# songhayeong/aes-fhe

Measured on AMD Instinct MI355X. Metric: AES-128 blocks/sec (homomorphic full round) at N=2^16, L=30; 1/2/4/8 MI355X, higher is better.
Workload: dtype u64

## Files before the change

aes-fhe_amd/csrc/bconv_cols.h:

```cpp
#pragma once
#include "bconv_mfma.h"
#include "ntt256f.h"

namespace aesfhe {

__device__ __forceinline__ void cols256_stages_store(double (&x)[16], double q, double qi, bool big, const double* tg,
                                                     const double* tws, double* s, u64* out, int b, int cl, int c) {
#pragma unroll
    for (int st = 0; st < 4; st++) {
        const int m = 1 << st, hh = 8 >> st;
        if (big && st == 2) {
#pragma unroll
            for (int a = 0; a < 16; a++) x[a] = fred(x[a], q, qi);
        }
#pragma unroll
        for (int a = 0; a < 16; a++) {
            if (a & hh) continue;
            const int ti = m + (a >> (4 - st));
            ct_f(x[a], x[a + hh], tg[ti], q, qi);
        }
    }
#pragma unroll
    for (int a = 0; a < 16; a++) s[(a * 16 + b) * kPadF + cl] = x[a];
    __syncthreads();
    const int ap = b;
#pragma unroll
    for (int bb = 0; bb < 16; bb++) x[bb] = s[(ap * 16 + bb) * kPadF + cl];
#pragma unroll
    for (int st = 4; st < 8; st++) {
        const int m = 1 << st, hh = 128 >> st;
        if (big && (st & 1) == 0) {
#pragma unroll
            for (int bb = 0; bb < 16; bb++) x[bb] = fred(x[bb], q, qi);
        }
#pragma unroll
        for (int bb = 0; bb < 16; bb++) {
            if (bb & hh) continue;
            ct_f(x[bb], x[bb + hh], tws[m + ap * (m >> 4) + (bb >> (8 - st))], q, qi);
        }
    }
#pragma unroll
    for (int bb = 0; bb < 16; bb++) st_d(&out[(ap * 16 + bb) * 256 + c], x[bb]);
}

template <int NSTEP, bool YIN, bool VC = false, int PF = 1, int TT = 4, int LT = 2, int MODE = 0>
__global__ __launch_bounds__(256, TT == 4 ? 2 : 3) void k_bconv_cols(BconvArgs a, Tabs T, int ntile) {
    static_assert(TT == 4 || TT == 2, "4 or 2 targets per workgroup");
    static_assert(LT == 1 || LT == 2, "1 or 2 LDS tiles");
    __shared__ double s[LT][256 * kPadF];
    __shared__ double tws[TT][256];
    const int tid = threadIdx.x, lane = tid & 63, w = tid >> 6, c = lane & 31, h = lane >> 5;
    const int cl = tid & 15, b = tid >> 4;
    const int id = blockIdx.x, x8 = id & 7, j = id >> 3;
    const int tile = j % ntile, u = (j / ntile) * 8 + x8;
    const int bx = u & 15, z = u >> 4, zb = z / a.nc, zc = z - zb * a.nc;
    const int logN = T.logN;
    const u64* src = a.src + (long)zb * a.sbs + (long)zc * a.scs;
    u64* dst = a.dst + (long)zb * a.dbs + (long)zc * a.dcs;
    auto limb_of = [&](int tau) { return tau < a.skip0 ? tau : tau + a.skipn; };
    auto pid_of = [&](int tl) { return tl <= a.tl_l ? tl : a.Lp1 + tl - a.tl_l - 1; };
    const int tau0 = TT * tile;
    const int nlive = min(TT, a.nt - tau0);
#pragma unroll
    for (int m = 0; m < TT; m++)
        if (m < nlive) tws[m][tid] = T.psid[((long)pid_of(limb_of(tau0 + m)) << logN) + tid];
    bc_v4i af[NSTEP];
    {
        const int row = lane & 31, ta = row >> 3, pb = (row & 3) + 4 * ((row >> 2) & 1);
        const int tau = tau0 + ta;
        const bc_v4i* ap =
            (const bc_v4i*)(a.tab + ((long)(ta < TT && tau < a.nt ? pid_of(limb_of(tau)) : 0) * 8 + pb) * kBconvKT + 16 * h);
#pragma unroll
        for (int st = 0; st < NSTEP; st++) af[st] = ap[2 * st];
    }
    const u64* sp[NSTEP][2];
    double sq[NSTEP][2], sf[NSTEP][2];
#pragma unroll
    for (int st = 0; st < NSTEP; st++)
#pragma unroll
        for (int uu = 0; uu < 2; uu++) {
            const int sl = 4 * st + 2 * h + uu;
            const int i = sl < a.ns ? sl : 0;
            sp[st][uu] = src + ((long)i << logN) + bx * 16 + (c & 15);
            if (!YIN) {
                const int pid = i < a.s_nq ? a.s_q0 + i : a.s_p0 + i - a.s_nq;
                sq[st][uu] = (double)a.qall[pid];
                sf[st][uu] = a.sinvf[i];
            }
        }
    double xv[TT][16];
    double eq[TT], eqi[TT], ew32[TT], ef32[TT], ecr[TT];
#pragma unroll
    for (int m = 0; m < TT; m++) {
        const int pid = tau0 + m < a.nt ? pid_of(limb_of(tau0 + m)) : 0;
        const double* pc = a.pc + 4 * pid;
        eq[m] = pc[0], eqi[m] = pc[1], ew32[m] = pc[2], ef32[m] = pc[3], ecr[m] = a.corr[pid];
    }
    double ev[VC ? 4 * NSTEP : 1];
#pragma unroll
    for (int sl = 0; sl < (VC ? 4 * NSTEP : 0); sl++) ev[sl] = a.einv[sl];
    u64 raw[PF + 1][NSTEP][2][2];
    auto load = [&](u64 (&r)[NSTEP][2][2], int ar) {
#pragma unroll
        for (int st = 0; st < NSTEP; st++)
#pragma unroll
            for (int uu = 0; uu < 2; uu++)
#pragma unroll
                for (int g = 0; g < 2; g++) r[st][uu][g] = sp[st][uu][(16 * ar + 4 * w + 2 * g + (c >> 4)) * 256];
    };
#pragma unroll
    for (int p = 0; p < PF; p++) load(raw[p], p);
#pragma unroll
    for (int ar = 0; ar < 16; ar++) {
        if (ar + PF < 16) load(raw[(ar + PF) % (PF + 1)], ar + PF);
        bc_v4i bf[2][NSTEP];
        double ys[2][NSTEP][2];
#pragma unroll
        for (int st = 0; st < NSTEP; st++)
#pragma unroll
            for (int uu = 0; uu < 2; uu++)
#pragma unroll
                for (int g = 0; g < 2; g++) {
                    u64 yb = PF ? raw[ar % (PF + 1)][st][uu][g] : sp[st][uu][(16 * ar + 4 * w + 2 * g + (c >> 4)) * 256];
                    if (!YIN) {
                        const double q = sq[st][uu], f = sf[st][uu];
                        double y = fmul_rem(u2d(yb), tw_w(f, q), f, q);
                        y = y < 0.0 ? y + q : y;
                        yb = (u64)__double_as_longlong(y + 4503599627370496.0) & 0xFFFFFFFFFFFFFULL;
                    }
                    if (VC) ys[g][st][uu] = u2d(yb);
                    bf[g][st][2 * uu] = (int)(unsigned)yb ^ (int)0x80808080;
                    bf[g][st][2 * uu + 1] = (int)(unsigned)(yb >> 32) ^ (int)0x80808080;
                }
        if constexpr (VC) {
            double yl[NSTEP][2][2];
#pragma unroll
            for (int st = 0; st < NSTEP; st++)
#pragma unroll
                for (int uu = 0; uu < 2; uu++) swap_halves(ys[0][st][uu], ys[1][st][uu], yl[st][uu][0], yl[st][uu][1]);
            double sum = 0.0;
#pragma unroll
            for (int st = 0; st < NSTEP; st++)
#pragma unroll
                for (int hh = 0; hh < 2; hh++)
#pragma unroll
                    for (int uu = 0; uu < 2; uu++) {
                        const int sl = 4 * st + 2 * hh + uu;
                        sum = sum + yl[st][uu][hh] * ev[sl];
                    }
            const int vown = (int)__builtin_rint(sum);
            const auto pr = __builtin_amdgcn_permlane32_swap((unsigned)vown, (unsigned)vown, false, false);
            const int voth = (int)(h ? pr[0] : pr[1]);
#pragma unroll
            for (int st = 0; st < NSTEP; st++)
#pragma unroll
                for (int uu = 0; uu < 2; uu++)
                    if (4 * st + 2 * h + uu == a.ns) {
#pragma unroll
                        for (int g = 0; g < 2; g++) {
                            bf[g][st][2 * uu] = ((g == h ? vown : voth) & 0xff) ^ (int)0x80808080;
                            bf[g][st][2 * uu + 1] = (int)0x80808080;
                        }
                    }
        }
        if constexpr (MODE == 2) {
#pragma unroll
            for (int m = 0; m < TT; m++) xv[m][ar] = (double)(bf[0][0][0] & 0xffffff) + (double)(bf[1][NSTEP - 1][3] & 0xff);
            continue;
        }
        bc_v16i acc[2];
#pragma unroll
        for (int g = 0; g < 2; g++) {
            acc[g] = bc_v16i{};
#pragma unroll
            for (int st = 0; st < NSTEP; st++) acc[g] = __builtin_amdgcn_mfma_i32_32x32x32_i8(af[st], bf[g][st], acc[g], 0, 0, 0);
        }
#pragma unroll
        for (int m = 0; m < TT; m++) {
            if (m >= nlive) break;
            double part[2];
#pragma unroll
            for (int g = 0; g < 2; g++) {
                const int p01 = acc[g][4 * m] + acc[g][4 * m + 1] * 256, p23 = acc[g][4 * m + 2] + acc[g][4 * m + 3] * 256;
                part[g] = __builtin_fma((double)p23, 65536.0, (double)p01);
            }
            double lo, hi;
            swap_halves(part[0], part[1], lo, hi);
            xv[m][ar] = fred(lo + fmul_rem(hi, ew32[m], ef32[m], eq[m]) + ecr[m], eq[m], eqi[m]);
        }
    }
    __syncthreads();
    if constexpr (MODE == 1) {
#pragma unroll
        for (int m = 0; m < TT; m++) {
            if (m >= nlive) break;
            u64* o = dst + ((long)limb_of(tau0 + m) << logN);
#pragma unroll
            for (int ar = 0; ar < 16; ar++) st_d(&o[(ar * 16 + b) * 256 + bx * 16 + cl], xv[m][ar]);
        }
        return;
    }
#pragma unroll
    for (int m = 0; m < TT; m++) {
        if (m >= nlive) break;
        if (LT == 1 && m > 0) __syncthreads();
        const int tl = limb_of(tau0 + m), pid = pid_of(tl);
        const double q = (double)T.q[pid], qi = T.qinv[pid];
        cols256_stages_store(xv[m], q, qi, q >= kBigPrime, T.psid + ((long)pid << logN), tws[m], s[m % LT],
                             dst + ((long)tl << logN), b, cl, bx * 16 + cl);
    }
}

}
```

aes-fhe_amd/csrc/ks_fused.h:

```cpp
#pragma once
#include "kernels_ops.h"
#include "ntt256f.h"

namespace aesfhe {

__device__ __forceinline__ int r8p(int e) { return e + (e >> 3); }

__device__ __forceinline__ void wave_lds_sync() {
    __builtin_amdgcn_fence(__ATOMIC_RELEASE, "wavefront");
    __builtin_amdgcn_wave_barrier();
    __builtin_amdgcn_fence(__ATOMIC_ACQUIRE, "wavefront");
}

__device__ __forceinline__ void row_ntt8_stages(double (&x)[8], double* sr, int L, int rt, const double* W, double q,
                                                double qi, bool big);
__device__ __forceinline__ void row_ntt8_fwd(double (&x)[8], const u64* rp, double* sr, int L, int rt,
                                             const double* W, double q, double qi, bool big) {
#pragma unroll
    for (int r = 0; r < 8; r++) x[r] = ld_d(&rp[L + 32 * r]);
    row_ntt8_stages(x, sr, L, rt, W, q, qi, big);
}
__device__ __forceinline__ void row_ntt8_stages(double (&x)[8], double* sr, int L, int rt, const double* W, double q,
                                                double qi, bool big) {
#pragma unroll
    for (int st = 0; st < 3; st++) {
        const int ml = 1 << st, h = 4 >> st;
        if (big && (st & 1) == 0) {
#pragma unroll
            for (int r = 0; r < 8; r++) x[r] = fred(x[r], q, qi);
        }
        const int base = ml * rt;
#pragma unroll
        for (int j = 0; j < ml; j++) {
            const double w = W[base + j];
#pragma unroll
            for (int k = 0; k < h; k++) ct_f(x[j * 2 * h + k], x[j * 2 * h + k + h], w, q, qi);
        }
    }
#pragma unroll
    for (int r = 0; r < 8; r++) sr[r8p(L + 32 * r)] = x[r];
    wave_lds_sync();
    const int eb = 32 * (L >> 2) + (L & 3);
#pragma unroll
    for (int r = 0; r < 8; r++) x[r] = sr[r8p(eb + 4 * r)];
#pragma unroll
    for (int st = 3; st < 6; st++) {
        const int ml = 1 << st, h = 4 >> (st - 3), nj = ml >> 3;
        if (big && (st & 1) == 0) {
#pragma unroll
            for (int r = 0; r < 8; r++) x[r] = fred(x[r], q, qi);
        }
        const int base = ml * rt + (L >> 2) * nj;
#pragma unroll
        for (int j = 0; j < nj; j++) {
            const double w = W[base + j];
#pragma unroll
            for (int k = 0; k < h; k++) ct_f(x[j * 2 * h + k], x[j * 2 * h + k + h], w, q, qi);
        }
    }
    wave_lds_sync();
#pragma unroll
    for (int r = 0; r < 8; r++) sr[r8p(eb + 4 * r)] = x[r];
    wave_lds_sync();
#pragma unroll
    for (int r = 0; r < 8; r++) x[r] = sr[r8p(8 * L + r)];
    if (big) {
#pragma unroll
        for (int r = 0; r < 8; r++) x[r] = fred(x[r], q, qi);
    }
    {
        const int base = 64 * rt + 2 * L;
        const double w0 = W[base], w1 = W[base + 1];
        ct_f(x[0], x[2], w0, q, qi);
        ct_f(x[1], x[3], w0, q, qi);
        ct_f(x[4], x[6], w1, q, qi);
        ct_f(x[5], x[7], w1, q, qi);
    }
    {
        const int base = 128 * rt + 4 * L;
#pragma unroll
        for (int j = 0; j < 4; j++) ct_f(x[2 * j], x[2 * j + 1], W[base + j], q, qi);
    }
    wave_lds_sync();
#pragma unroll
    for (int r = 0; r < 8; r++) sr[r8p(8 * L + r)] = big ? fred(x[r], q, qi) : x[r];
    wave_lds_sync();
#pragma unroll
    for (int r = 0; r < 8; r++) x[r] = sr[r8p(L + 32 * r)];
    wave_lds_sync();
}

__device__ __forceinline__ void row_intt8(double (&x)[8], double* sr, int L, const double* W, double q, double qi,
                                          bool big) {
    auto gs = [&](double& a, double& b, double w) {
        if (big) gs_f<true>(a, b, w, q, qi);
        else gs_f<false>(a, b, w, q, qi);
    };
#pragma unroll
    for (int r = 0; r < 8; r++) sr[r8p(L + 32 * r)] = x[r];
    wave_lds_sync();
#pragma unroll
    for (int r = 0; r < 8; r++) x[r] = sr[r8p(8 * L + r)];
#pragma unroll
    for (int j = 0; j < 4; j++) gs(x[2 * j], x[2 * j + 1], W[128 + 4 * L + j]);
    {
        const double w0 = W[64 + 2 * L], w1 = W[64 + 2 * L + 1];
        gs(x[0], x[2], w0);
        gs(x[1], x[3], w0);
        gs(x[4], x[6], w1);
        gs(x[5], x[7], w1);
    }
    wave_lds_sync();
#pragma unroll
    for (int r = 0; r < 8; r++) sr[r8p(8 * L + r)] = x[r];
    wave_lds_sync();
    const int eb = 32 * (L >> 2) + (L & 3);
#pragma unroll
    for (int r = 0; r < 8; r++) x[r] = sr[r8p(eb + 4 * r)];
#pragma unroll
    for (int st = 5; st >= 3; st--) {
        const int ml = 1 << st, h = 4 >> (st - 3), nj = ml >> 3;
        const int base = ml + (L >> 2) * nj;
#pragma unroll
        for (int j = 0; j < nj; j++) {
            const double w = W[base + j];
#pragma unroll
            for (int k = 0; k < h; k++) gs(x[j * 2 * h + k], x[j * 2 * h + k + h], w);
        }
    }
    wave_lds_sync();
#pragma unroll
    for (int r = 0; r < 8; r++) sr[r8p(eb + 4 * r)] = x[r];
    wave_lds_sync();
#pragma unroll
    for (int r = 0; r < 8; r++) x[r] = sr[r8p(L + 32 * r)];
#pragma unroll
    for (int st = 2; st >= 0; st--) {
        const int ml = 1 << st, h = 4 >> st;
#pragma unroll
        for (int j = 0; j < ml; j++) {
            const double w = W[ml + j];
#pragma unroll
            for (int k = 0; k < h; k++) gs(x[j * 2 * h + k], x[j * 2 * h + k + h], w);
        }
    }
    wave_lds_sync();
}

template <bool FMA>
__device__ __forceinline__ void ks_prod_prologue(double (&a0)[8], double (&a1)[8], const u64* kp, long kcomp,
                                                 const u64* xa, long aps, const u64* xb, long bps, const u64* xc,
                                                 long cps, bool has_c, double wv, double f, double fal, double fC,
                                                 double fK, double q, double qi, bool big) {
    double x0[8], x1[8], y0[8], y1[8], kb[8], ka[8];
#pragma unroll
    for (int r = 0; r < 8; r++) {
        x0[r] = u2d(xa[32 * r]);
        x1[r] = u2d(xa[aps + 32 * r]);
        y0[r] = u2d(xb[32 * r]);
        y1[r] = u2d(xb[bps + 32 * r]);
        kb[r] = u2d(kp[32 * r]);
        ka[r] = u2d(kp[32 * r + kcomp]);
    }
#pragma unroll
    for (int r = 0; r < 8; r++) {
        double p0 = fmul_remq(x0[r], y0[r], qi, q);
        double p1 = fmul_remq(x0[r], y1[r], qi, q) + fmul_remq(x1[r], y0[r], qi, q);
        double p2 = fmul_remq(x1[r], y1[r], qi, q);
        if constexpr (FMA) {
            p0 = fmul_remq(p0, fal, qi, q) + fK;
            p1 = fmul_remq(p1, fal, qi, q);
            p2 = fmul_remq(p2, fal, qi, q);
            if (has_c) {
                p0 += fmul_remq(u2d(xc[32 * r]), fC, qi, q);
                p1 += fmul_remq(u2d(xc[cps + 32 * r]), fC, qi, q);
            }
        }
        a0[r] = fmul_rem(p0, wv, f, q) + fmul_remq(p2, kb[r], qi, q);
        a1[r] = fmul_rem(p1, wv, f, q) + fmul_remq(p2, ka[r], qi, q);
        if (big) {
            a0[r] = fred(a0[r], q, qi);
            a1[r] = fred(a1[r], q, qi);
        }
    }
}

struct KsFin {
    const u64* conv;
    long cbs, cps;
    u64* out;
    long obs, ops;
    const double* dinvf;
    Opnd2 add;
};
template <int G, int R = 256, bool PROD = false, int EPI = 0>
__global__ __launch_bounds__(256, 4) void k_nttf_rows_ks(const u64* __restrict__ d, long dbs,
                                                      const u64* __restrict__ ext, long exs, long exj,
                                                      const u64* __restrict__ key, long kdig, long kcomp,
                                                      u64* __restrict__ acc, long abs_, long acs, int B,
                                                      int beta, int K, int l, int ne, Tabs T, Opnd addend,
                                                      const double* __restrict__ pmodf, int accum, Opnd pb,
                                                      const u64* __restrict__ fac, Opnd pc, int t0, int nt,
                                                      KsFin fin) {
    static_assert(G == 1 && !PROD && EPI == 0, "the accumulating giants' kernel: the other forms are k_nttf_rows_ks_p's");
    __shared__ double s[8 * 288 + 8 * 256];
    const int nbg = (B + G - 1) / G;
    const int id = blockIdx.x, x8 = id & 7, rest = id >> 3;
    const int b0 = (rest % nbg) * G, pair = (rest / nbg) * 8 + x8;
    constexpr int RB = R / 8;
    constexpr int LOGN = R == 256 ? 16 : 17;
    const int tq = pair / RB, rb = pair - tq * RB;
    if (tq >= nt) return;
    const int t = t0 + tq;
    const int pid = t <= l ? t : T.Lp1 + (t - l - 1);
    const int own = t <= l ? t / K : -1;
    const int tid = threadIdx.x, L = tid & 31, rl = tid >> 5;
    const int row = rb * 8 + rl;
    const double q = (double)T.q[pid], qi = T.qinv[pid];
    const bool big = q >= kBigPrime;
    const double* W = T.psid + ((long)pid << LOGN);
    double* sr = s + rl * 288;
    double* tw = s + 8 * 288 + rl * 256;
#pragma unroll
    for (int m = 0; m < 8; m++) {
        const int e = L + 32 * m;
        if (e > 0) {
            const int ml = 1 << (31 - __clz(e));
            tw[e] = W[(long)ml * (R + row) + (e - ml)];
        }
    }
    wave_lds_sync();
    const long roff = ((long)t << LOGN) + (long)row * 256 + L;
    double a0[G][8], a1[G][8];
#pragma unroll
    for (int g = 0; g < G; g++) {
        const int bb = b0 + g;
#pragma unroll
        for (int r = 0; r < 8; r++) a0[g][r] = a1[g][r] = 0.0;
        if (bb >= B) continue;
        if (pmodf && t <= l && addend.ptr) {
            const double f = pmodf[t], w = tw_w(f, q);
            const u64* xa = addend.ptr + (long)bb * addend.bs + roff;
            if (addend.np > 0) {
#pragma unroll
                for (int r = 0; r < 8; r++) a0[g][r] = fmul_rem(u2d(xa[32 * r]), w, f, q);
            }
            if (addend.np > 1) {
#pragma unroll
                for (int r = 0; r < 8; r++) a1[g][r] = fmul_rem(u2d(xa[addend.ps + 32 * r]), w, f, q);
            }
        }
        if (accum) {
            const u64* o0 = acc + (long)bb * abs_ + roff;
#pragma unroll
            for (int r = 0; r < 8; r++) {
                a0[g][r] = fred(a0[g][r] + u2d(o0[32 * r]), q, qi);
                a1[g][r] = fred(a1[g][r] + u2d(o0[acs + 32 * r]), q, qi);
            }
        }
    }
    int nsum = 0;
#pragma unroll 1
    for (int j = 0; j < beta; j++) {
        const u64* kp = key + (long)j * kdig + ((long)pid << LOGN) + (long)row * 256 + L;
        u64 kbw[8], kaw[8];
#pragma unroll
        for (int r = 0; r < 8; r++) {
            kbw[r] = kp[32 * r];
            kaw[r] = kp[32 * r + kcomp];
        }
#pragma unroll
        for (int g = 0; g < G; g++) {
            const int bb = b0 + g;
            if (bb >= B) break;
            double v[8];
            if (j == own) {
                const u64* dp = d + (long)bb * dbs + roff;
#pragma unroll
                for (int r = 0; r < 8; r++) v[r] = u2d(dp[32 * r]);
            } else {
                row_ntt8_fwd(v, ext + (long)j * exj + (long)bb * exs + ((long)t << LOGN) + (long)row * 256, sr, L, 1,
                             tw, q, qi, big);
            }
#pragma unroll
            for (int r = 0; r < 8; r++) {
                const double kb = u2d(kbw[r]), ka = u2d(kaw[r]);
                a0[g][r] += fmul_remq(v[r], kb, qi, q);
                a1[g][r] += fmul_remq(v[r], ka, qi, q);
            }
        }
        if (big && (++nsum & 3) == 0) {
#pragma unroll
            for (int g = 0; g < G; g++)
#pragma unroll
                for (int r = 0; r < 8; r++) {
                    a0[g][r] = fred(a0[g][r], q, qi);
                    a1[g][r] = fred(a1[g][r], q, qi);
                }
        }
    }
#pragma unroll
    for (int g = 0; g < G; g++) {
        const int bb = b0 + g;
        if (bb >= B) break;
        u64* o0 = acc + (long)bb * abs_ + roff;
#pragma unroll
        for (int r = 0; r < 8; r++) {
            __builtin_nontemporal_store(fcanon(a0[g][r], q, qi), &o0[32 * r]);
            __builtin_nontemporal_store(fcanon(a1[g][r], q, qi), &o0[acs + 32 * r]);
        }
    }
}

typedef __attribute__((address_space(3))) void ks_lds_void;
__device__ __forceinline__ void ks_dma_rows(const u64* g, double* lds_wave, int lane) {
#pragma unroll
    for (int k = 0; k < 4; k++)
        __builtin_amdgcn_global_load_lds((const void*)(g + 128 * k + 2 * lane), (ks_lds_void*)(lds_wave + 128 * k), 16, 0, 0);
}
__device__ __forceinline__ void ks_dma_wait() {
    asm volatile("s_waitcnt vmcnt(0)" ::: "memory");
    __builtin_amdgcn_wave_barrier();
}
__device__ __forceinline__ void ks_lds_reads_done() {
    asm volatile("s_waitcnt lgkmcnt(0)" ::: "memory");
    __builtin_amdgcn_wave_barrier();
}

template <int R = 256, bool PROD = false, int EPI = 0>
__global__ __launch_bounds__(256, 3) void k_nttf_rows_ks_p(const u64* __restrict__ d, long dbs,
                                                      const u64* __restrict__ ext, long exs, long exj,
                                                      const u64* __restrict__ key, long kdig, long kcomp,
                                                      u64* __restrict__ acc, long abs_, long acs, int B,
                                                      int beta, int K, int l, int ne, Tabs T, Opnd addend,
                                                      const double* __restrict__ pmodf, int accum, Opnd pb,
                                                      const u64* __restrict__ fac, Opnd pc, int t0, int nt,
                                                      KsFin fin) {
    static_assert(EPI == 1 || EPI == 2, "FIN or INV: the canonical accumulators are k_nttf_rows_ks's");
    constexpr bool FIN = EPI == 1;
    __shared__ double s[8 * 288 + 8 * 256 + 8 * 256];
    const int id = blockIdx.x, x8 = id & 7, rest = id >> 3;
    const int bb = rest % B, pair = (rest / B) * 8 + x8;
    constexpr int RB = R / 8;
    constexpr int LOGN = R == 256 ? 16 : 17;
    const int tq = pair / RB, rb = pair - tq * RB;
    if (tq >= nt) return;
    const int t = t0 + tq;
    const int pid = t <= l ? t : T.Lp1 + (t - l - 1);
    const int own = t <= l ? t / K : -1;
    const int tid = threadIdx.x, L = tid & 31, rl = tid >> 5, lane = tid & 63, w = tid >> 6;
    const int row = rb * 8 + rl;
    const double q = (double)T.q[pid], qi = T.qinv[pid];
    const bool big = q >= kBigPrime;
    const double* W = T.psid + ((long)pid << LOGN);
    double* sr = s + rl * 288;
    double* tw = s + 8 * 288 + rl * 256;
    double* ebw = s + 8 * 288 + 8 * 256 + w * 512;
    const double* er = ebw + (rl & 1) * 256;
    const long woff = ((long)t << LOGN) + (long)(rb * 8 + 2 * w) * 256;
    auto next_digit = [&](int j) {
        for (j++; j < beta && j == own; j++) {
        }
        return j;
    };
    int jn = next_digit(-1);
    if (jn < beta) ks_dma_rows(ext + (long)jn * exj + (long)bb * exs + woff, ebw, lane);
#pragma unroll
    for (int m = 0; m < 8; m++) {
        const int e = L + 32 * m;
        if (e > 0) {
            const int ml = 1 << (31 - __clz(e));
            tw[e] = W[(long)ml * (R + row) + (e - ml)];
        }
    }
    const long roff = ((long)t << LOGN) + (long)row * 256 + L;
    double a0[8], a1[8];
#pragma unroll
    for (int r = 0; r < 8; r++) a0[r] = a1[r] = 0.0;
    if (PROD && t <= l) {
        const double f = pmodf[t], wv = tw_w(f, q);
        const u64* kp = key + (long)own * kdig + ((long)pid << LOGN) + (long)row * 256 + L;
        const u64* xa = addend.ptr + (long)(bb & addend.bmask) * addend.bs + roff;
        const u64* xb = pb.ptr + (long)(bb & pb.bmask) * pb.bs + roff;
        const u64* xc = pc.ptr ? pc.ptr + (long)(bb & pc.bmask) * pc.bs + roff : xb;
        if (fac)
            ks_prod_prologue<true>(a0, a1, kp, kcomp, xa, addend.ps, xb, pb.ps, xc, pc.ps, pc.ptr != nullptr, wv, f,
                                   (double)fac[3 * t], (double)fac[3 * t + 1], (double)fac[3 * t + 2], q, qi, big);
        else
            ks_prod_prologue<false>(a0, a1, kp, kcomp, xa, addend.ps, xb, pb.ps, xc, pc.ps, false, wv, f, 0.0, 0.0, 0.0,
                                    q, qi, big);
    } else if (!PROD) {
        if (pmodf && t <= l && addend.ptr) {
            const double f = pmodf[t], wv = tw_w(f, q);
            const u64* xa = addend.ptr + (long)bb * addend.bs + roff;
            if (addend.np > 0) {
#pragma unroll
                for (int r = 0; r < 8; r++) a0[r] = fmul_rem(u2d(xa[32 * r]), wv, f, q);
            }
            if (addend.np > 1) {
#pragma unroll
                for (int r = 0; r < 8; r++) a1[r] = fmul_rem(u2d(xa[addend.ps + 32 * r]), wv, f, q);
            }
        }
        if (own >= 0 && own < beta) {
            const u64* kp = key + (long)own * kdig + ((long)pid << LOGN) + (long)row * 256 + L;
            const u64* dp = d + (long)bb * dbs + roff;
#pragma unroll
            for (int r = 0; r < 8; r++) {
                const double v = u2d(dp[32 * r]), kb = u2d(kp[32 * r]), ka = u2d(kp[32 * r + kcomp]);
                a0[r] += fmul_remq(v, kb, qi, q);
                a1[r] += fmul_remq(v, ka, qi, q);
            }
        }
    }
    if (accum) {
        const u64* o0 = acc + (long)bb * abs_ + roff;
#pragma unroll
        for (int r = 0; r < 8; r++) {
            a0[r] = fred(a0[r] + u2d(o0[32 * r]), q, qi);
            a1[r] = fred(a1[r] + u2d(o0[acs + 32 * r]), q, qi);
        }
    } else if (big) {
#pragma unroll
        for (int r = 0; r < 8; r++) {
            a0[r] = fred(a0[r], q, qi);
            a1[r] = fred(a1[r], q, qi);
        }
    }
    wave_lds_sync();
    int nsum = 0;
    const long coff = ((long)t << LOGN) + (long)(rb * 8 + 2 * w) * 256;
#pragma unroll 1
    while (jn < beta) {
        const int j = jn;
        ks_dma_wait();
        double v[8];
#pragma unroll
        for (int r = 0; r < 8; r++) v[r] = er[L + 32 * r];
        ks_lds_reads_done();
        jn = next_digit(j);
        if (jn < beta) ks_dma_rows(ext + (long)jn * exj + (long)bb * exs + woff, ebw, lane);
        else if (FIN) ks_dma_rows(fin.conv + (long)bb * fin.cbs + coff, ebw, lane);
        const u64* kp = key + (long)j * kdig + ((long)pid << LOGN) + (long)row * 256 + L;
        u64 kbw[8], kaw[8];
#pragma unroll
        for (int r = 0; r < 8; r++) {
            kbw[r] = kp[32 * r];
            kaw[r] = kp[32 * r + kcomp];
        }
        row_ntt8_stages(v, sr, L, 1, tw, q, qi, big);
#pragma unroll
        for (int r = 0; r < 8; r++) {
            const double kb = u2d(kbw[r]), ka = u2d(kaw[r]);
            a0[r] += fmul_remq(v[r], kb, qi, q);
            a1[r] += fmul_remq(v[r], ka, qi, q);
        }
        if (big && (++nsum & 3) == 0) {
#pragma unroll
            for (int r = 0; r < 8; r++) {
                a0[r] = fred(a0[r], q, qi);
                a1[r] = fred(a1[r], q, qi);
            }
        }
    }
    if constexpr (FIN) {
        const double f = fin.dinvf[t], wv = tw_w(f, q);
        if (beta == 0 || next_digit(-1) >= beta)
            ks_dma_rows(fin.conv + (long)bb * fin.cbs + coff, ebw, lane);
#pragma unroll 1
        for (int c = 0; c < 2; c++) {
            ks_dma_wait();
            double cv[8];
#pragma unroll
            for (int r = 0; r < 8; r++) cv[r] = er[L + 32 * r];
            ks_lds_reads_done();
            if (c == 0) ks_dma_rows(fin.conv + (long)bb * fin.cbs + fin.cps + coff, ebw, lane);
            row_ntt8_stages(cv, sr, L, 1, tw, q, qi, big);
            const u64* ap = fin.add.ptr && c < fin.add.np ? fin.add.ptr + (long)bb * fin.add.bs + (long)c * fin.add.ps + roff
                                                          : nullptr;
            u64* op = fin.out + (long)bb * fin.obs + (long)c * fin.ops + roff;
#pragma unroll
            for (int r = 0; r < 8; r++) {
                double a = c ? a1[r] : a0[r];
                if (big) a = fred(a, q, qi);
                double v = fmul_rem(a - cv[r], wv, f, q);
                if (ap) v += u2d(ap[32 * r]);
                __builtin_nontemporal_store(fcanon(v, q, qi), &op[32 * r]);
            }
        }
        return;
    }
    const double* IW = T.ipsid + ((long)pid << LOGN);
#pragma unroll
    for (int m = 0; m < 8; m++) {
        const int e = L + 32 * m;
        if (e > 0) {
            const int ml = 1 << (31 - __clz(e));
            tw[e] = IW[(long)ml * (R + row) + (e - ml)];
        }
    }
    wave_lds_sync();
    u64* o0 = acc + (long)bb * abs_ + roff;
#pragma unroll
    for (int c = 0; c < 2; c++) {
        double x[8];
#pragma unroll
        for (int r = 0; r < 8; r++) x[r] = fred(c ? a1[r] : a0[r], q, qi);
        row_intt8(x, sr, L, tw, q, qi, big);
#pragma unroll
        for (int r = 0; r < 8; r++) st_d(&o0[(long)c * acs + 32 * r], x[r]);
    }
}

}
```

Before: 284,000.

## Specialize key-switch and bconv kernels on compile-time big-prime and guard flags

Turns the runtime big-prime flag in the fused key-switch kernel into a compile-time type, so the whole body is instantiated twice and the per-butterfly and per-accumulation branches fold away. The bconv column kernel gets a GUARD template parameter that picks, when all targets are live, a path without the per-target liveness check. The prologue is specialised on the FMA and has-addend flags, the key loads are reordered for the FMA form, next_digit loses its loop, and the final store's addend check moves out of the row loop. Duplicating the bodies grows code size and may raise register pressure or instruction-cache load.

```diff
diff --git a/aes-fhe_amd/csrc/bconv_cols.h b/aes-fhe_amd/csrc/bconv_cols.h
--- a/aes-fhe_amd/csrc/bconv_cols.h
+++ b/aes-fhe_amd/csrc/bconv_cols.h
@@ -1,6 +1,8 @@
 #pragma once
 #include "bconv_mfma.h"
 #include "ntt256f.h"
+
+#include <type_traits>
 
 namespace aesfhe {
 
@@ -43,7 +45,7 @@
     for (int bb = 0; bb < 16; bb++) st_d(&out[(ap * 16 + bb) * 256 + c], x[bb]);
 }
 
-template <int NSTEP, bool YIN, bool VC = false, int PF = 1, int TT = 4, int LT = 2, int MODE = 0>
+template <int NSTEP, bool YIN, bool VC = false, int PF = 1, int TT = 4, int LT = 2, int MODE = 0, int GUARD = 2>
 __global__ __launch_bounds__(256, TT == 4 ? 2 : 3) void k_bconv_cols(BconvArgs a, Tabs T, int ntile) {
     static_assert(TT == 4 || TT == 2, "4 or 2 targets per workgroup");
     static_assert(LT == 1 || LT == 2, "1 or 2 LDS tiles");
@@ -108,87 +110,93 @@
 #pragma unroll
                 for (int g = 0; g < 2; g++) r[st][uu][g] = sp[st][uu][(16 * ar + 4 * w + 2 * g + (c >> 4)) * 256];
     };
-#pragma unroll
-    for (int p = 0; p < PF; p++) load(raw[p], p);
-#pragma unroll
-    for (int ar = 0; ar < 16; ar++) {
-        if (ar + PF < 16) load(raw[(ar + PF) % (PF + 1)], ar + PF);
-        bc_v4i bf[2][NSTEP];
-        double ys[2][NSTEP][2];
-#pragma unroll
-        for (int st = 0; st < NSTEP; st++)
-#pragma unroll
-            for (int uu = 0; uu < 2; uu++)
+    auto convert = [&](auto guarded) {
+#pragma unroll
+        for (int p = 0; p < PF; p++) load(raw[p], p);
+#pragma unroll
+        for (int ar = 0; ar < 16; ar++) {
+            if (ar + PF < 16) load(raw[(ar + PF) % (PF + 1)], ar + PF);
+            bc_v4i bf[2][NSTEP];
+            double ys[2][NSTEP][2];
+#pragma unroll
+            for (int st = 0; st < NSTEP; st++)
+#pragma unroll
+                for (int uu = 0; uu < 2; uu++)
+#pragma unroll
+                    for (int g = 0; g < 2; g++) {
+                        u64 yb = PF ? raw[ar % (PF + 1)][st][uu][g] : sp[st][uu][(16 * ar + 4 * w + 2 * g + (c >> 4)) * 256];
+                        if (!YIN) {
+                            const double q = sq[st][uu], f = sf[st][uu];
+                            double y = fmul_rem(u2d(yb), tw_w(f, q), f, q);
+                            y = y < 0.0 ? y + q : y;
+                            yb = (u64)__double_as_longlong(y + 4503599627370496.0) & 0xFFFFFFFFFFFFFULL;
+                        }
+                        if (VC) ys[g][st][uu] = u2d(yb);
+                        bf[g][st][2 * uu] = (int)(unsigned)yb ^ (int)0x80808080;
+                        bf[g][st][2 * uu + 1] = (int)(unsigned)(yb >> 32) ^ (int)0x80808080;
+                    }
+            if constexpr (VC) {
+                double yl[NSTEP][2][2];
+#pragma unroll
+                for (int st = 0; st < NSTEP; st++)
+#pragma unroll
+                    for (int uu = 0; uu < 2; uu++) swap_halves(ys[0][st][uu], ys[1][st][uu], yl[st][uu][0], yl[st][uu][1]);
+                double sum = 0.0;
+#pragma unroll
+                for (int st = 0; st < NSTEP; st++)
+#pragma unroll
+                    for (int hh = 0; hh < 2; hh++)
+#pragma unroll
+                        for (int uu = 0; uu < 2; uu++) {
+                            const int sl = 4 * st + 2 * hh + uu;
+                            sum = sum + yl[st][uu][hh] * ev[sl];
+                        }
+                const int vown = (int)__builtin_rint(sum);
+                const auto pr = __builtin_amdgcn_permlane32_swap((unsigned)vown, (unsigned)vown, false, false);
+                const int voth = (int)(h ? pr[0] : pr[1]);
+#pragma unroll
+                for (int st = 0; st < NSTEP; st++)
+#pragma unroll
+                    for (int uu = 0; uu < 2; uu++)
+                        if (4 * st + 2 * h + uu == a.ns) {
+#pragma unroll
+                            for (int g = 0; g < 2; g++) {
+                                bf[g][st][2 * uu] = ((g == h ? vown : voth) & 0xff) ^ (int)0x80808080;
+                                bf[g][st][2 * uu + 1] = (int)0x80808080;
+                            }
+                        }
+            }
+            if constexpr (MODE == 2) {
+#pragma unroll
+                for (int m = 0; m < TT; m++) xv[m][ar] = (double)(bf[0][0][0] & 0xffffff) + (double)(bf[1][NSTEP - 1][3] & 0xff);
+                continue;
+            }
+            bc_v16i acc[2];
+#pragma unroll
+            for (int g = 0; g < 2; g++) {
+                acc[g] = bc_v16i{};
+#pragma unroll
+                for (int st = 0; st < NSTEP; st++) acc[g] = __builtin_amdgcn_mfma_i32_32x32x32_i8(af[st], bf[g][st], acc[g], 0, 0, 0);
+            }
+#pragma unroll
+            for (int m = 0; m < TT; m++) {
+                if (decltype(guarded)::value && m >= nlive) break;
+                double part[2];
 #pragma unroll
                 for (int g = 0; g < 2; g++) {
-                    u64 yb = PF ? raw[ar % (PF + 1)][st][uu][g] : sp[st][uu][(16 * ar + 4 * w + 2 * g + (c >> 4)) * 256];
-                    if (!YIN) {
-                        const double q = sq[st][uu], f = sf[st][uu];
-                        double y = fmul_rem(u2d(yb), tw_w(f, q), f, q);
-                        y = y < 0.0 ? y + q : y;
-                        yb = (u64)__double_as_longlong(y + 4503599627370496.0) & 0xFFFFFFFFFFFFFULL;
-                    }
-                    if (VC) ys[g][st][uu] = u2d(yb);
-                    bf[g][st][2 * uu] = (int)(unsigned)yb ^ (int)0x80808080;
-                    bf[g][st][2 * uu + 1] = (int)(unsigned)(yb >> 32) ^ (int)0x80808080;
+                    const int p01 = acc[g][4 * m] + acc[g][4 * m + 1] * 256, p23 = acc[g][4 * m + 2] + acc[g][4 * m + 3] * 256;
+                    part[g] = __builtin_fma((double)p23, 65536.0, (double)p01);
                 }
-        if constexpr (VC) {
-            double yl[NSTEP][2][2];
-#pragma unroll
-            for (int st = 0; st < NSTEP; st++)
-#pragma unroll
-                for (int uu = 0; uu < 2; uu++) swap_halves(ys[0][st][uu], ys[1][st][uu], yl[st][uu][0], yl[st][uu][1]);
-            double sum = 0.0;
-#pragma unroll
-            for (int st = 0; st < NSTEP; st++)
-#pragma unroll
-                for (int hh = 0; hh < 2; hh++)
-#pragma unroll
-                    for (int uu = 0; uu < 2; uu++) {
-                        const int sl = 4 * st + 2 * hh + uu;
-                        sum = sum + yl[st][uu][hh] * ev[sl];
-                    }
-            const int vown = (int)__builtin_rint(sum);
-            const auto pr = __builtin_amdgcn_permlane32_swap((unsigned)vown, (unsigned)vown, false, false);
-            const int voth = (int)(h ? pr[0] : pr[1]);
-#pragma unroll
-            for (int st = 0; st < NSTEP; st++)
-#pragma unroll
-                for (int uu = 0; uu < 2; uu++)
-                    if (4 * st + 2 * h + uu == a.ns) {
-#pragma unroll
-                        for (int g = 0; g < 2; g++) {
-                            bf[g][st][2 * uu] = ((g == h ? vown : voth) & 0xff) ^ (int)0x80808080;
-                            bf[g][st][2 * uu + 1] = (int)0x80808080;
-                        }
-                    }
-        }
-        if constexpr (MODE == 2) {
-#pragma unroll
-            for (int m = 0; m < TT; m++) xv[m][ar] = (double)(bf[0][0][0] & 0xffffff) + (double)(bf[1][NSTEP - 1][3] & 0xff);
-            continue;
-        }
-        bc_v16i acc[2];
-#pragma unroll
-        for (int g = 0; g < 2; g++) {
-            acc[g] = bc_v16i{};
-#pragma unroll
-            for (int st = 0; st < NSTEP; st++) acc[g] = __builtin_amdgcn_mfma_i32_32x32x32_i8(af[st], bf[g][st], acc[g], 0, 0, 0);
-        }
-#pragma unroll
-        for (int m = 0; m < TT; m++) {
-            if (m >= nlive) break;
-            double part[2];
-#pragma unroll
-            for (int g = 0; g < 2; g++) {
-                const int p01 = acc[g][4 * m] + acc[g][4 * m + 1] * 256, p23 = acc[g][4 * m + 2] + acc[g][4 * m + 3] * 256;
-                part[g] = __builtin_fma((double)p23, 65536.0, (double)p01);
-            }
-            double lo, hi;
-            swap_halves(part[0], part[1], lo, hi);
-            xv[m][ar] = fred(lo + fmul_rem(hi, ew32[m], ef32[m], eq[m]) + ecr[m], eq[m], eqi[m]);
-        }
-    }
+                double lo, hi;
+                swap_halves(part[0], part[1], lo, hi);
+                xv[m][ar] = fred(lo + fmul_rem(hi, ew32[m], ef32[m], eq[m]) + ecr[m], eq[m], eqi[m]);
+            }
+        }
+    };
+    if constexpr (GUARD == 0) convert(std::false_type{});
+    else if constexpr (GUARD == 1) convert(std::true_type{});
+    else if (nlive == TT) convert(std::false_type{});
+    else convert(std::true_type{});
     __syncthreads();
     if constexpr (MODE == 1) {
 #pragma unroll
diff --git a/aes-fhe_amd/csrc/ks_fused.h b/aes-fhe_amd/csrc/ks_fused.h
--- a/aes-fhe_amd/csrc/ks_fused.h
+++ b/aes-fhe_amd/csrc/ks_fused.h
@@ -1,6 +1,8 @@
 #pragma once
 #include "kernels_ops.h"
 #include "ntt256f.h"
+
+#include <type_traits>
 
 namespace aesfhe {
 
@@ -12,16 +14,20 @@
     __builtin_amdgcn_fence(__ATOMIC_ACQUIRE, "wavefront");
 }
 
+template <bool BIG>
+using KsBig = std::integral_constant<bool, BIG>;
+template <class Big>
 __device__ __forceinline__ void row_ntt8_stages(double (&x)[8], double* sr, int L, int rt, const double* W, double q,
-                                                double qi, bool big);
+                                                double qi, Big big);
 __device__ __forceinline__ void row_ntt8_fwd(double (&x)[8], const u64* rp, double* sr, int L, int rt,
                                              const double* W, double q, double qi, bool big) {
 #pragma unroll
     for (int r = 0; r < 8; r++) x[r] = ld_d(&rp[L + 32 * r]);
     row_ntt8_stages(x, sr, L, rt, W, q, qi, big);
 }
+template <class Big>
 __device__ __forceinline__ void row_ntt8_stages(double (&x)[8], double* sr, int L, int rt, const double* W, double q,
-                                                double qi, bool big) {
+                                                double qi, Big big) {
 #pragma unroll
     for (int st = 0; st < 3; st++) {
         const int ml = 1 << st, h = 4 >> st;
@@ -90,25 +96,21 @@
     wave_lds_sync();
 }
 
-__device__ __forceinline__ void row_intt8(double (&x)[8], double* sr, int L, const double* W, double q, double qi,
-                                          bool big) {
-    auto gs = [&](double& a, double& b, double w) {
-        if (big) gs_f<true>(a, b, w, q, qi);
-        else gs_f<false>(a, b, w, q, qi);
-    };
+template <bool BIG>
+__device__ __forceinline__ void row_intt8(double (&x)[8], double* sr, int L, const double* W, double q, double qi) {
 #pragma unroll
     for (int r = 0; r < 8; r++) sr[r8p(L + 32 * r)] = x[r];
     wave_lds_sync();
 #pragma unroll
     for (int r = 0; r < 8; r++) x[r] = sr[r8p(8 * L + r)];
 #pragma unroll
-    for (int j = 0; j < 4; j++) gs(x[2 * j], x[2 * j + 1], W[128 + 4 * L + j]);
+    for (int j = 0; j < 4; j++) gs_f<BIG>(x[2 * j], x[2 * j + 1], W[128 + 4 * L + j], q, qi);
     {
         const double w0 = W[64 + 2 * L], w1 = W[64 + 2 * L + 1];
-        gs(x[0], x[2], w0);
-        gs(x[1], x[3], w0);
-        gs(x[4], x[6], w1);
-        gs(x[5], x[7], w1);
+        gs_f<BIG>(x[0], x[2], w0, q, qi);
+        gs_f<BIG>(x[1], x[3], w0, q, qi);
+        gs_f<BIG>(x[4], x[6], w1, q, qi);
+        gs_f<BIG>(x[5], x[7], w1, q, qi);
     }
     wave_lds_sync();
 #pragma unroll
@@ -125,7 +127,7 @@
         for (int j = 0; j < nj; j++) {
             const double w = W[base + j];
 #pragma unroll
-            for (int k = 0; k < h; k++) gs(x[j * 2 * h + k], x[j * 2 * h + k + h], w);
+            for (int k = 0; k < h; k++) gs_f<BIG>(x[j * 2 * h + k], x[j * 2 * h + k + h], w, q, qi);
         }
     }
     wave_lds_sync();
@@ -141,17 +143,18 @@
         for (int j = 0; j < ml; j++) {
             const double w = W[ml + j];
 #pragma unroll
-            for (int k = 0; k < h; k++) gs(x[j * 2 * h + k], x[j * 2 * h + k + h], w);
-        }
-    }
-    wave_lds_sync();
-}
-
-template <bool FMA>
+            for (int k = 0; k < h; k++) gs_f<BIG>(x[j * 2 * h + k], x[j * 2 * h + k + h], w, q, qi);
+        }
+    }
+    wave_lds_sync();
+}
+
+template <bool FMA, bool HAS_C, bool BIG>
 __device__ __forceinline__ void ks_prod_prologue(double (&a0)[8], double (&a1)[8], const u64* kp, long kcomp,
                                                  const u64* xa, long aps, const u64* xb, long bps, const u64* xc,
-                                                 long cps, bool has_c, double wv, double f, double fal, double fC,
-                                                 double fK, double q, double qi, bool big) {
+                                                 long cps, double wv, double f, double fal, double fC, double fK,
+                                                 double q, double qi) {
+    static_assert(FMA || !HAS_C, "the addend ciphertext belongs to the multiply-add form");
     double x0[8], x1[8], y0[8], y1[8], kb[8], ka[8];
 #pragma unroll
     for (int r = 0; r < 8; r++) {
@@ -159,11 +162,17 @@
         x1[r] = u2d(xa[aps + 32 * r]);
         y0[r] = u2d(xb[32 * r]);
         y1[r] = u2d(xb[bps + 32 * r]);
-        kb[r] = u2d(kp[32 * r]);
-        ka[r] = u2d(kp[32 * r + kcomp]);
+        if constexpr (!FMA) {
+            kb[r] = u2d(kp[32 * r]);
+            ka[r] = u2d(kp[32 * r + kcomp]);
+        }
     }
 #pragma unroll
     for (int r = 0; r < 8; r++) {
+        if constexpr (FMA) {
+            kb[r] = u2d(kp[32 * r]);
+            ka[r] = u2d(kp[32 * r + kcomp]);
+        }
         double p0 = fmul_remq(x0[r], y0[r], qi, q);
         double p1 = fmul_remq(x0[r], y1[r], qi, q) + fmul_remq(x1[r], y0[r], qi, q);
         double p2 = fmul_remq(x1[r], y1[r], qi, q);
@@ -171,14 +180,14 @@
             p0 = fmul_remq(p0, fal, qi, q) + fK;
             p1 = fmul_remq(p1, fal, qi, q);
             p2 = fmul_remq(p2, fal, qi, q);
-            if (has_c) {
+            if constexpr (HAS_C) {
                 p0 += fmul_remq(u2d(xc[32 * r]), fC, qi, q);
                 p1 += fmul_remq(u2d(xc[cps + 32 * r]), fC, qi, q);
             }
         }
         a0[r] = fmul_rem(p0, wv, f, q) + fmul_remq(p2, kb[r], qi, q);
         a1[r] = fmul_rem(p1, wv, f, q) + fmul_remq(p2, ka[r], qi, q);
-        if (big) {
+        if constexpr (BIG) {
             a0[r] = fred(a0[r], q, qi);
             a1[r] = fred(a1[r], q, qi);
         }
@@ -351,18 +360,13 @@
     const int tid = threadIdx.x, L = tid & 31, rl = tid >> 5, lane = tid & 63, w = tid >> 6;
     const int row = rb * 8 + rl;
     const double q = (double)T.q[pid], qi = T.qinv[pid];
-    const bool big = q >= kBigPrime;
     const double* W = T.psid + ((long)pid << LOGN);
     double* sr = s + rl * 288;
     double* tw = s + 8 * 288 + rl * 256;
     double* ebw = s + 8 * 288 + 8 * 256 + w * 512;
     const double* er = ebw + (rl & 1) * 256;
     const long woff = ((long)t << LOGN) + (long)(rb * 8 + 2 * w) * 256;
-    auto next_digit = [&](int j) {
-        for (j++; j < beta && j == own; j++) {
-        }
-        return j;
-    };
+    auto next_digit = [&](int j) { return j + 1 == own ? j + 2 : j + 1; };
     int jn = next_digit(-1);
     if (jn < beta) ks_dma_rows(ext + (long)jn * exj + (long)bb * exs + woff, ebw, lane);
 #pragma unroll
@@ -374,142 +378,161 @@
         }
     }
     const long roff = ((long)t << LOGN) + (long)row * 256 + L;
-    double a0[8], a1[8];
-#pragma unroll
-    for (int r = 0; r < 8; r++) a0[r] = a1[r] = 0.0;
-    if (PROD && t <= l) {
-        const double f = pmodf[t], wv = tw_w(f, q);
-        const u64* kp = key + (long)own * kdig + ((long)pid << LOGN) + (long)row * 256 + L;
-        const u64* xa = addend.ptr + (long)(bb & addend.bmask) * addend.bs + roff;
-        const u64* xb = pb.ptr + (long)(bb & pb.bmask) * pb.bs + roff;
-        const u64* xc = pc.ptr ? pc.ptr + (long)(bb & pc.bmask) * pc.bs + roff : xb;
-        if (fac)
-            ks_prod_prologue<true>(a0, a1, kp, kcomp, xa, addend.ps, xb, pb.ps, xc, pc.ps, pc.ptr != nullptr, wv, f,
-                                   (double)fac[3 * t], (double)fac[3 * t + 1], (double)fac[3 * t + 2], q, qi, big);
-        else
-            ks_prod_prologue<false>(a0, a1, kp, kcomp, xa, addend.ps, xb, pb.ps, xc, pc.ps, false, wv, f, 0.0, 0.0, 0.0,
-                                    q, qi, big);
-    } else if (!PROD) {
-        if (pmodf && t <= l && addend.ptr) {
+    auto body = [&](auto big) {
+        constexpr bool BIG = decltype(big)::value;
+        double a0[8], a1[8];
+#pragma unroll
+        for (int r = 0; r < 8; r++) a0[r] = a1[r] = 0.0;
+        if (PROD && t <= l) {
             const double f = pmodf[t], wv = tw_w(f, q);
-            const u64* xa = addend.ptr + (long)bb * addend.bs + roff;
-            if (addend.np > 0) {
-#pragma unroll
-                for (int r = 0; r < 8; r++) a0[r] = fmul_rem(u2d(xa[32 * r]), wv, f, q);
-            }
-            if (addend.np > 1) {
-#pragma unroll
-                for (int r = 0; r < 8; r++) a1[r] = fmul_rem(u2d(xa[addend.ps + 32 * r]), wv, f, q);
-            }
-        }
-        if (own >= 0 && own < beta) {
             const u64* kp = key + (long)own * kdig + ((long)pid << LOGN) + (long)row * 256 + L;
-            const u64* dp = d + (long)bb * dbs + roff;
+            const u64* xa = addend.ptr + (long)(bb & addend.bmask) * addend.bs + roff;
+            const u64* xb = pb.ptr + (long)(bb & pb.bmask) * pb.bs + roff;
+            const u64* xc = pc.ptr ? pc.ptr + (long)(bb & pc.bmask) * pc.bs + roff : xb;
+            if (fac) {
+                const double fal = (double)fac[3 * t], fC = (double)fac[3 * t + 1], fK = (double)fac[3 * t + 2];
+                if (pc.ptr)
+                    ks_prod_prologue<true, true, BIG>(a0, a1, kp, kcomp, xa, addend.ps, xb, pb.ps, xc, pc.ps, wv, f, fal, fC,
+                                                      fK, q, qi);
+                else
+                    ks_prod_prologue<true, false, BIG>(a0, a1, kp, kcomp, xa, addend.ps, xb, pb.ps, xc, pc.ps, wv, f, fal,
+                                                       fC, fK, q, qi);
+            } else {
+                ks_prod_prologue<false, false, BIG>(a0, a1, kp, kcomp, xa, addend.ps, xb, pb.ps, xc, pc.ps, wv, f, 0.0, 0.0,
+                                                    0.0, q, qi);
+            }
+        } else if (!PROD) {
+            if (pmodf && t <= l && addend.ptr) {
+                const double f = pmodf[t], wv = tw_w(f, q);
+                const u64* xa = addend.ptr + (long)bb * addend.bs + roff;
+                if (addend.np > 0) {
+#pragma unroll
+                    for (int r = 0; r < 8; r++) a0[r] = fmul_rem(u2d(xa[32 * r]), wv, f, q);
+                }
+                if (addend.np > 1) {
+#pragma unroll
+                    for (int r = 0; r < 8; r++) a1[r] = fmul_rem(u2d(xa[addend.ps + 32 * r]), wv, f, q);
+                }
+            }
+            if (own >= 0 && own < beta) {
+                const u64* kp = key + (long)own * kdig + ((long)pid << LOGN) + (long)row * 256 + L;
+                const u64* dp = d + (long)bb * dbs + roff;
+#pragma unroll
+                for (int r = 0; r < 8; r++) {
+                    const double v = u2d(dp[32 * r]), kb = u2d(kp[32 * r]), ka = u2d(kp[32 * r + kcomp]);
+                    a0[r] += fmul_remq(v, kb, qi, q);
+                    a1[r] += fmul_remq(v, ka, qi, q);
+                }
+            }
+        }
+        if (accum) {
+            const u64* o0 = acc + (long)bb * abs_ + roff;
 #pragma unroll
             for (int r = 0; r < 8; r++) {
-                const double v = u2d(dp[32 * r]), kb = u2d(kp[32 * r]), ka = u2d(kp[32 * r + kcomp]);
-                a0[r] += fmul_remq(v, kb, qi, q);
-                a1[r] += fmul_remq(v, ka, qi, q);
-            }
-        }
-    }
-    if (accum) {
-        const u64* o0 = acc + (long)bb * abs_ + roff;
-#pragma unroll
-        for (int r = 0; r < 8; r++) {
-            a0[r] = fred(a0[r] + u2d(o0[32 * r]), q, qi);
-            a1[r] = fred(a1[r] + u2d(o0[acs + 32 * r]), q, qi);
-        }
-    } else if (big) {
-#pragma unroll
-        for (int r = 0; r < 8; r++) {
-            a0[r] = fred(a0[r], q, qi);
-            a1[r] = fred(a1[r], q, qi);
-        }
-    }
-    wave_lds_sync();
-    int nsum = 0;
-    const long coff = ((long)t << LOGN) + (long)(rb * 8 + 2 * w) * 256;
-#pragma unroll 1
-    while (jn < beta) {
-        const int j = jn;
-        ks_dma_wait();
-        double v[8];
-#pragma unroll
-        for (int r = 0; r < 8; r++) v[r] = er[L + 32 * r];
-        ks_lds_reads_done();
-        jn = next_digit(j);
-        if (jn < beta) ks_dma_rows(ext + (long)jn * exj + (long)bb * exs + woff, ebw, lane);
-        else if (FIN) ks_dma_rows(fin.conv + (long)bb * fin.cbs + coff, ebw, lane);
-        const u64* kp = key + (long)j * kdig + ((long)pid << LOGN) + (long)row * 256 + L;
-        u64 kbw[8], kaw[8];
-#pragma unroll
-        for (int r = 0; r < 8; r++) {
-            kbw[r] = kp[32 * r];
-            kaw[r] = kp[32 * r + kcomp];
-        }
-        row_ntt8_stages(v, sr, L, 1, tw, q, qi, big);
-#pragma unroll
-        for (int r = 0; r < 8; r++) {
-            const double kb = u2d(kbw[r]), ka = u2d(kaw[r]);
-            a0[r] += fmul_remq(v[r], kb, qi, q);
-            a1[r] += fmul_remq(v[r], ka, qi, q);
-        }
-        if (big && (++nsum & 3) == 0) {
+                a0[r] = fred(a0[r] + u2d(o0[32 * r]), q, qi);
+                a1[r] = fred(a1[r] + u2d(o0[acs + 32 * r]), q, qi);
+            }
+        } else if (BIG) {
 #pragma unroll
             for (int r = 0; r < 8; r++) {
                 a0[r] = fred(a0[r], q, qi);
                 a1[r] = fred(a1[r], q, qi);
             }
         }
-    }
-    if constexpr (FIN) {
-        const double f = fin.dinvf[t], wv = tw_w(f, q);
-        if (beta == 0 || next_digit(-1) >= beta)
-            ks_dma_rows(fin.conv + (long)bb * fin.cbs + coff, ebw, lane);
+        wave_lds_sync();
+        int nsum = 0;
+        const long coff = ((long)t << LOGN) + (long)(rb * 8 + 2 * w) * 256;
 #pragma unroll 1
+        while (jn < beta) {
+            const int j = jn;
+            ks_dma_wait();
+            double v[8];
+#pragma unroll
+            for (int r = 0; r < 8; r++) v[r] = er[L + 32 * r];
+            ks_lds_reads_done();
+            jn = next_digit(j);
+            if constexpr (FIN)
+                ks_dma_rows(jn < beta ? ext + (long)jn * exj + (long)bb * exs + woff : fin.conv + (long)bb * fin.cbs + coff,
+                            ebw, lane);
+            else if (jn < beta) ks_dma_rows(ext + (long)jn * exj + (long)bb * exs + woff, ebw, lane);
+            const u64* kp = key + (long)j * kdig + ((long)pid << LOGN) + (long)row * 256 + L;
+            u64 kbw[8], kaw[8];
+#pragma unroll
+            for (int r = 0; r < 8; r++) {
+                kbw[r] = kp[32 * r];
+                kaw[r] = kp[32 * r + kcomp];
+            }
+            row_ntt8_stages(v, sr, L, 1, tw, q, qi, big);
+#pragma unroll
+            for (int r = 0; r < 8; r++) {
+                const double kb = u2d(kbw[r]), ka = u2d(kaw[r]);
+                a0[r] += fmul_remq(v[r], kb, qi, q);
+                a1[r] += fmul_remq(v[r], ka, qi, q);
+            }
+            if (BIG && (++nsum & 3) == 0) {
+#pragma unroll
+                for (int r = 0; r < 8; r++) {
+                    a0[r] = fred(a0[r], q, qi);
+                    a1[r] = fred(a1[r], q, qi);
+                }
+            }
+        }
+        if constexpr (FIN) {
+            const double f = fin.dinvf[t], wv = tw_w(f, q);
+            if (beta == 0 || next_digit(-1) >= beta)
+                ks_dma_rows(fin.conv + (long)bb * fin.cbs + coff, ebw, lane);
+#pragma unroll 1
+            for (int c = 0; c < 2; c++) {
+                ks_dma_wait();
+                double cv[8];
+#pragma unroll
+                for (int r = 0; r < 8; r++) cv[r] = er[L + 32 * r];
+                ks_lds_reads_done();
+                if (c == 0) ks_dma_rows(fin.conv + (long)bb * fin.cbs + fin.cps + coff, ebw, lane);
+                row_ntt8_stages(cv, sr, L, 1, tw, q, qi, big);
+                const u64* ap = fin.add.ptr && c < fin.add.np ? fin.add.ptr + (long)bb * fin.add.bs + (long)c * fin.add.ps + roff
+                                                              : nullptr;
+                u64* op = fin.out + (long)bb * fin.obs + (long)c * fin.ops + roff;
+                double v[8];
+#pragma unroll
+                for (int r = 0; r < 8; r++) {
+                    double a = c ? a1[r] : a0[r];
+                    if constexpr (BIG) a = fred(a, q, qi);
+                    v[r] = fmul_rem(a - cv[r], wv, f, q);
+                }
+                if (ap) {
+#pragma unroll
+                    for (int r = 0; r < 8; r++) __builtin_nontemporal_store(fcanon(v[r] + u2d(ap[32 * r]), q, qi), &op[32 * r]);
+                } else {
+#pragma unroll
+                    for (int r = 0; r < 8; r++) __builtin_nontemporal_store(fcanon(v[r], q, qi), &op[32 * r]);
+                }
+            }
+            return;
+        }
+        const double* IW = T.ipsid + ((long)pid << LOGN);
+#pragma unroll
+        for (int m = 0; m < 8; m++) {
+            const int e = L + 32 * m;
+            if (e > 0) {
+                const int ml = 1 << (31 - __clz(e));
+                tw[e] = IW[(long)ml * (R + row) + (e - ml)];
+            }
+        }
+        wave_lds_sync();
+        u64* o0 = acc + (long)bb * abs_ + roff;
+#pragma unroll
         for (int c = 0; c < 2; c++) {
-            ks_dma_wait();
-            double cv[8];
-#pragma unroll
-            for (int r = 0; r < 8; r++) cv[r] = er[L + 32 * r];
-            ks_lds_reads_done();
-            if (c == 0) ks_dma_rows(fin.conv + (long)bb * fin.cbs + fin.cps + coff, ebw, lane);
-            row_ntt8_stages(cv, sr, L, 1, tw, q, qi, big);
-            const u64* ap = fin.add.ptr && c < fin.add.np ? fin.add.ptr + (long)bb * fin.add.bs + (long)c * fin.add.ps + roff
-                                                          : nullptr;
-            u64* op = fin.out + (long)bb * fin.obs + (long)c * fin.ops + roff;
-#pragma unroll
-            for (int r = 0; r < 8; r++) {
-                double a = c ? a1[r] : a0[r];
-                if (big) a = fred(a, q, qi);
-                double v = fmul_rem(a - cv[r], wv, f, q);
-                if (ap) v += u2d(ap[32 * r]);
-                __builtin_nontemporal_store(fcanon(v, q, qi), &op[32 * r]);
-            }
-        }
-        return;
-    }
-    const double* IW = T.ipsid + ((long)pid << LOGN);
-#pragma unroll
-    for (int m = 0; m < 8; m++) {
-        const int e = L + 32 * m;
-        if (e > 0) {
-            const int ml = 1 << (31 - __clz(e));
-            tw[e] = IW[(long)ml * (R + row) + (e - ml)];
-        }
-    }
-    wave_lds_sync();
-    u64* o0 = acc + (long)bb * abs_ + roff;
-#pragma unroll
-    for (int c = 0; c < 2; c++) {
-        double x[8];
-#pragma unroll
-        for (int r = 0; r < 8; r++) x[r] = fred(c ? a1[r] : a0[r], q, qi);
-        row_intt8(x, sr, L, tw, q, qi, big);
-#pragma unroll
-        for (int r = 0; r < 8; r++) st_d(&o0[(long)c * acs + 32 * r], x[r]);
-    }
-}
-
-}
+            double x[8];
+#pragma unroll
+            for (int r = 0; r < 8; r++) x[r] = fred(c ? a1[r] : a0[r], q, qi);
+            row_intt8<BIG>(x, sr, L, tw, q, qi);
+#pragma unroll
+            for (int r = 0; r < 8; r++) st_d(&o0[(long)c * acs + 32 * r], x[r]);
+        }
+    };
+    if (q >= kBigPrime) body(KsBig<true>{});
+    else body(KsBig<false>{});
+}
+
+}
```

Measured after the change: 287,000, median of 6. 1.01x the previous value.
